# wangjunchi/LLMSeg

Hardware: AMD Instinct MI355X
Metric: images/sec (1024x1024, 64-tok prompt) model_forward fwd+bwd (higher is better)
Workload: dtype bf16; 1 GPU; BASELINE.json configs[2]: synthetic 1024x1024 + random-init LLaVA-7B(Llama-7B+CLIP-L/14)/SAM-ViT-H, batch_size=2 per GPU, fwd+bwd train step (CE + align + IoP losses, LoRA r=8 dropout 0.05 on q/v + trainable embed/lm_head/text_fcs/lisa_*, frozen towers, fp32 gradient arena, AdamW step every 10 micro-steps inside the timed region, micro-step replayed from a hipGraph), 256 candidate masks, 64-token ; global_batch=2, parallelism=dp1, graph=True, valid=True

## Files before the change

include/llmseg_hip.h:

```cpp
#ifndef LLMSEG_HIP_H
#define LLMSEG_HIP_H

#include <stdint.h>

#ifdef __cplusplus
extern "C" {
#endif

#define LLMSEG_OK 0
#define LLMSEG_EINVAL (-1)
#define LLMSEG_ELAUNCH (-2)
#define LLMSEG_NOT_TAKEN 1

enum { LLMSEG_ACT_NONE = 0, LLMSEG_ACT_RELU = 1, LLMSEG_ACT_GELU = 2, LLMSEG_ACT_QUICKGELU = 3, LLMSEG_ACT_SILU = 4,
       LLMSEG_ACT_SIGMOID = 5 };

#define LLMSEG_ABI_VERSION 14

#define LLMSEG_REDUCE_WS_BYTES (16 << 20)
int llmseg_version(void);
int64_t llmseg_launch_count(void);
int64_t llmseg_struct_size(int which);
const char* llmseg_last_error(void);

typedef struct {
  uint32_t struct_size;
  uint32_t reserved0;
  const void* A; const void* W; void* C;
  const void* bias;
  const void* gamma;
  const void* residual;
  int64_t M, N, K;
  int64_t lda, ldw, ldc, ldr;
  int64_t batch, strideA, strideW, strideC;
  float alpha;
  int act;
  int out_f32;
  int trans_a;
  int trans_w;
  int64_t batch2, strideA2, strideW2, strideC2;
  const void* A2; const void* W2; int64_t lda2, ldw2;
  void* workspace; int64_t workspace_bytes;
  int accumulate;
  const void* a_norm_w; float a_norm_eps; int a_swiglu;
  const void* norm_w; float norm_eps; int reserved1; void* norm_out; int64_t ldn;
  int fx; int fx_T; int64_t fx_cols; const float* fx_cos; const float* fx_sin; void* fx_out; const void* fx_in; int64_t fx_ld;
  const void* nb_x; const void* nb_w; const void* nb_dres; float nb_eps; int nb_rms;
  const void* nb_lora_t; int64_t nb_lora_ldt; const void* nb_lora_w0; const void* nb_lora_w1; float nb_lora_alpha; int reserved2; const void* nb_lora_drop;
  const void* dl_o; int64_t dl_ldo; float* dl_out; int32_t dl_heads; int32_t dl_T;
  const float* nb_lora_part; int32_t nb_lora_S; float nb_lora_scale; int32_t nb_lora_zero; int32_t reserved3;
// ... 161 lines not shown
                      int32_t* n_chars, int32_t cap_chars, void* workspace, int64_t workspace_bytes, void* stream);
int64_t llmseg_rle_parse_ws_bytes(int32_t K, int64_t total_chars);
int llmseg_rle_parse(const uint8_t* chars, const int64_t* char_offsets, int32_t K, uint32_t* run_ends, int64_t* run_offsets, void* workspace,
                     int64_t workspace_bytes, void* stream);

int llmseg_colsum(const void* x, float* out, int64_t M, int64_t N, int64_t ld, void* workspace, int64_t workspace_bytes, void* stream);
int llmseg_norm_bwd(const void* dy, const void* x, const void* w, void* dx, float* dw, float* db, int64_t rows, int64_t cols,
                    float eps, int rms, void* workspace, int64_t workspace_bytes, void* stream);
int llmseg_norm_bwd_add(const void* dy, const void* x, const void* w, const void* dres, void* dx, float* dw, float* db, int64_t rows, int64_t cols,
                        float eps, int rms, void* workspace, int64_t workspace_bytes, void* stream);
int llmseg_swiglu_bwd(const void* gu, const void* dout, void* dgu, int64_t rows, int64_t I, void* stream);
int llmseg_act_bwd(const void* dy, const void* y, void* out, int64_t n, int act, void* stream);
int llmseg_linear_bwd(const void* dy, const void* y, int act, const void* x, const void* w, void* dx, float* dw, float* db, int64_t M, int64_t N, int64_t K,
                      int accumulate, void* stream);
int llmseg_softmax_rows(const float* S, void* P, int64_t BH, int32_t Tq, int32_t Tk, int32_t ld, float scale, int32_t causal,
                        const uint8_t* key_mask, int32_t heads, void* stream);
int llmseg_attn_ds(const void* P, const float* dP, void* dS, int64_t rows, int32_t T, int32_t ld, float scale, void* stream);
int llmseg_ce_bwd(const void* logits, const int64_t* labels, const float* coef, void* dlogits, int32_t N, int32_t T, int64_t V,
                  int64_t ldl, void* stream);
int llmseg_scatter_add_rows(const void* src, const int64_t* idx, float* dst, int64_t n, int64_t cols, void* stream);
typedef struct {
  const uint64_t* rng_state;
  uint32_t stream;
  uint32_t drop_thr;
  uint32_t seg_rows;
  uint32_t reserved0;
} llmseg_dropout;
int llmseg_lora_down(const void* x0, const void* x1, int64_t ldx, const void* w0, const void* w1, void* y, int64_t ldy, int64_t M, int64_t K,
                     int32_t w_kr, float alpha, int32_t zero_cols, const llmseg_dropout* drop, void* stream);
int llmseg_lora_down_ws(const void* x0, const void* x1, int64_t ldx, const void* w0, const void* w1, void* y, int64_t ldy, int64_t M, int64_t K,
                        int32_t w_kr, float alpha, int32_t zero_cols, const llmseg_dropout* drop, void* scratch, int64_t scratch_bytes, void* stream);
int llmseg_lora_outer(const void* a0, const void* a1, int64_t lda, const void* b0, const void* b1, int64_t ldb, float* out0, float* out1, int64_t M,
                      int64_t N, int32_t out_rn, float alpha, const llmseg_dropout* drop, void* workspace, int64_t workspace_bytes, void* stream);
int llmseg_lora_wgrads(const void* dq, const void* dv, int64_t ldd, const void* x, int64_t ldx, const void* xa, int64_t ldxa, const void* t, int64_t ldt,
                       float* gbq, float* gbv, float* gaq, float* gav, int64_t M, int64_t H, float s, const llmseg_dropout* drop, void* workspace,
                       int64_t workspace_bytes, void* stream);
int llmseg_lora_apply(void* y, int64_t ldy, const void* xa, int64_t ldxa, const void* w0, const void* w1, int64_t M, int64_t N, int32_t w_rn,
                      float alpha, const llmseg_dropout* drop, void* stream);
int llmseg_lora_pack(const void* aq, const void* bq, const void* av, const void* bv, void* w2b, void* w2a, void* bt, int64_t H, float s, void* stream);
int llmseg_lora_down_parts(const void* x0, const void* x1, int64_t ldx, const void* w0, const void* w1, void* y, int64_t ldy, int64_t M, int64_t K,
                           int32_t w_kr, float alpha, int32_t zero_cols, const llmseg_dropout* drop, void* scratch, int64_t scratch_bytes, int32_t* S_out,
                           float* scale_out, void* stream);
int llmseg_lora_down_pack(const void* x0, const void* x1, int64_t ldx, const void* w0, const void* w1, void* y, int64_t ldy, int64_t M, int64_t K,
                          int32_t w_kr, float alpha, int32_t zero_cols, const llmseg_dropout* drop, void* scratch, int64_t scratch_bytes, const void* aq,
                          const void* bq, const void* av, const void* bv, void* w2b, void* w2a, void* bt, int64_t H, float s, void* stream);
int llmseg_transpose_pad(const void* in, void* out, int64_t rows, int64_t cols, int64_t ld_in, int64_t ld_out, int64_t rows_pad, void* stream);
int llmseg_sumsq(const void* x, int64_t n, int is_f32, float* out, void* workspace, int64_t workspace_bytes, void* stream);
int llmseg_adamw(void* p, float* master, const void* grad, int grad_f32, float* m, float* v, int64_t n, float lr, float beta1,
                 float beta2, float eps, float weight_decay, int64_t step, const float* grad_scale, void* stream);

int llmseg_prof_enable(int on);
const char* llmseg_prof_dominant_kernel(void);
double llmseg_prof_dominant_bytes(void);
int llmseg_prof_dominant_info(int64_t* out4);
int llmseg_prof_collect(double* total_ms, double* total_flops, int64_t* launches, double* dom_ms, double* dom_flops, int64_t* dom_launches);

#ifdef __cplusplus
}
#endif
#endif
```

llmseg_amd/_lib.py:

```python
import ctypes as C
import os

_HERE = os.path.dirname(os.path.abspath(__file__))
LIB_PATH = os.environ.get("LLMSEG_LIB") or os.path.join(_HERE, "libllmseg_hip.so")

ABI_VERSION = 14

ACT_NONE, ACT_RELU, ACT_GELU, ACT_QUICKGELU, ACT_SILU, ACT_SIGMOID = range(6)
NOT_TAKEN = 1


class _Sized(C.Structure):

    def __init__(self, *a, **kw):
        super().__init__(*a, **kw)
        self.struct_size = C.sizeof(self)


class GemmArgs(_Sized):
    _fields_ = [("struct_size", C.c_uint32), ("reserved0", C.c_uint32), ("A", C.c_void_p), ("W", C.c_void_p), ("C", C.c_void_p),
                ("bias", C.c_void_p), ("gamma", C.c_void_p), ("residual", C.c_void_p),
                ("M", C.c_int64), ("N", C.c_int64), ("K", C.c_int64),
                ("lda", C.c_int64), ("ldw", C.c_int64), ("ldc", C.c_int64), ("ldr", C.c_int64),
                ("batch", C.c_int64), ("strideA", C.c_int64), ("strideW", C.c_int64), ("strideC", C.c_int64),
                ("alpha", C.c_float), ("act", C.c_int), ("out_f32", C.c_int), ("trans_a", C.c_int), ("trans_w", C.c_int),
                ("batch2", C.c_int64), ("strideA2", C.c_int64), ("strideW2", C.c_int64), ("strideC2", C.c_int64),
                ("A2", C.c_void_p), ("W2", C.c_void_p), ("lda2", C.c_int64), ("ldw2", C.c_int64),
                ("workspace", C.c_void_p), ("workspace_bytes", C.c_int64), ("accumulate", C.c_int),
                ("a_norm_w", C.c_void_p), ("a_norm_eps", C.c_float), ("a_swiglu", C.c_int),
                ("norm_w", C.c_void_p), ("norm_eps", C.c_float), ("reserved1", C.c_int), ("norm_out", C.c_void_p), ("ldn", C.c_int64),
                ("fx", C.c_int), ("fx_T", C.c_int), ("fx_cols", C.c_int64), ("fx_cos", C.c_void_p), ("fx_sin", C.c_void_p), ("fx_out", C.c_void_p),
                ("fx_in", C.c_void_p), ("fx_ld", C.c_int64),
                ("nb_x", C.c_void_p), ("nb_w", C.c_void_p), ("nb_dres", C.c_void_p), ("nb_eps", C.c_float), ("nb_rms", C.c_int),
                ("nb_lora_t", C.c_void_p), ("nb_lora_ldt", C.c_int64), ("nb_lora_w0", C.c_void_p), ("nb_lora_w1", C.c_void_p), ("nb_lora_alpha", C.c_float),
                ("reserved2", C.c_int), ("nb_lora_drop", C.c_void_p),
                ("dl_o", C.c_void_p), ("dl_ldo", C.c_int64), ("dl_out", C.c_void_p), ("dl_heads", C.c_int32), ("dl_T", C.c_int32),
                ("nb_lora_part", C.c_void_p), ("nb_lora_S", C.c_int32), ("nb_lora_scale", C.c_float), ("nb_lora_zero", C.c_int32), ("reserved3", C.c_int32)]

class GemmW8Args(_Sized):
# ... 78 lines not shown
    "llmseg_cosine_scores": [_p, _p, _p, _i32, _i32, _p],
    "llmseg_linear_f32": [_p, _i64, _p, _i64, _i32, _p, _p, _i64, _p, _i64, _i32, _i32, _i32, _i32, _f32, _p],
    "llmseg_layernorm_f32": [_p, _p, _p, _p, _i64, _i32, _f32, _p],
    "llmseg_attn_f32": [_p, _p, _p, _p, C.POINTER(C.c_int64), _i32, _i32, _i32, _i32, _i32, _f32, _p],
    "llmseg_cosine_f32": [_p, _p, _p, _i32, _i32, _p],
    "llmseg_align_reg_loss": [_p, _p, _p, _p, _p, _p, _p, _p, _p, _i32, _i32, _f32, _i32, _p],
    "llmseg_dice_bce": [_p, _p, _p, _i32, _i64, _f32, _p, _i64, _p],
    "llmseg_dice_bce_bwd": [_p, _p, _p, _p, _i32, _i64, _f32, _p],
    "llmseg_ce_loss": [_p, _p, _p, _i32, _i32, _i64, _i64, _p, _i64, _p],
    "llmseg_intersection_union": [_p, _p, _i64, _i32, _p, _p],
    "llmseg_union_resize_iou": [_p, _p, _p, _i32, _i32, _i32, _i32, _i32, _i32, _i32, _i32, _p, _p],
    "llmseg_rle_decode": [_p, _p, _p, _i32, _i32, _i32, _i32, _p],
    "llmseg_rle_encode_ws_bytes": [_i32, _i32, _i32],
    "llmseg_rle_encode": [_p, _i32, _i32, _i32, _p, _p, _i32, _p, _p, _i32, _p, _i64, _p],
    "llmseg_rle_parse_ws_bytes": [_i32, _i64],
    "llmseg_rle_parse": [_p, _p, _i32, _p, _p, _p, _i64, _p],
    "llmseg_mask_targets": [_p, _p, _p, _p, _i32, _i32, _i32, _i32, _i32, _p, _p, _p, _p, _p],
    "llmseg_gt_resample": [_p, _p, _p, _p, _i32, _i32, _i32, _i32, _p],
    "llmseg_proposal_targets": [_p, _p, _p, _i32, _p, _i32, _i32, _i32, _i32, _p, _p, _p, _p, _p, _p, _i32, _p, _p, _p, _p, _p],
    "llmseg_resize_aa": [_p, _p, _i32, _i32, _i32, _i32, _p, _p, _p, _p, _p, _p, _i32, _p],
    "llmseg_colsum": [_p, _p, _i64, _i64, _i64, _p, _i64, _p],
    "llmseg_norm_bwd": [_p, _p, _p, _p, _p, _p, _i64, _i64, _f32, C.c_int, _p, _i64, _p],
    "llmseg_norm_bwd_add": [_p, _p, _p, _p, _p, _p, _p, _i64, _i64, _f32, C.c_int, _p, _i64, _p],
    "llmseg_swiglu_bwd": [_p, _p, _p, _i64, _i64, _p],
    "llmseg_act_bwd": [_p, _p, _p, _i64, C.c_int, _p],
    "llmseg_linear_bwd": [_p, _p, C.c_int, _p, _p, _p, _p, _p, _i64, _i64, _i64, C.c_int, _p],
    "llmseg_softmax_rows": [_p, _p, _i64, _i32, _i32, _i32, _f32, _i32, _p, _i32, _p],
    "llmseg_attn_ds": [_p, _p, _p, _i64, _i32, _i32, _f32, _p],
    "llmseg_ce_bwd": [_p, _p, _p, _p, _i32, _i32, _i64, _i64, _p],
    "llmseg_scatter_add_rows": [_p, _p, _p, _i64, _i64, _p],
    "llmseg_lora_down": [_p, _p, _i64, _p, _p, _p, _i64, _i64, _i64, _i32, _f32, _i32, _dp, _p],
    "llmseg_lora_down_ws": [_p, _p, _i64, _p, _p, _p, _i64, _i64, _i64, _i32, _f32, _i32, _dp, _p, _i64, _p],
    "llmseg_lora_outer": [_p, _p, _i64, _p, _p, _i64, _p, _p, _i64, _i64, _i32, _f32, _dp, _p, _i64, _p],
    "llmseg_lora_wgrads": [_p, _p, _i64, _p, _i64, _p, _i64, _p, _i64, _p, _p, _p, _p, _i64, _i64, _f32, _dp, _p, _i64, _p],
    "llmseg_lora_apply": [_p, _i64, _p, _i64, _p, _p, _i64, _i64, _i32, _f32, _dp, _p],
    "llmseg_lora_pack": [_p, _p, _p, _p, _p, _p, _p, _i64, _f32, _p],
    "llmseg_lora_down_parts": [_p, _p, _i64, _p, _p, _p, _i64, _i64, _i64, _i32, _f32, _i32, _dp, _p, _i64, C.POINTER(C.c_int32), C.POINTER(C.c_float), _p],
    "llmseg_lora_down_pack": [_p, _p, _i64, _p, _p, _p, _i64, _i64, _i64, _i32, _f32, _i32, _dp, _p, _i64, _p, _p, _p, _p, _p, _p, _p, _i64, _f32, _p],
    "llmseg_transpose_pad": [_p, _p, _i64, _i64, _i64, _i64, _i64, _p],
    "llmseg_sumsq": [_p, _i64, C.c_int, _p, _p, _i64, _p],
    "llmseg_adamw": [_p, _p, _p, C.c_int, _p, _p, _i64, _f32, _f32, _f32, _f32, _f32, _i64, _p, _p],
    "llmseg_prof_enable": [C.c_int],
    "llmseg_prof_dominant_kernel": [],
    "llmseg_prof_dominant_bytes": [],
    "llmseg_prof_dominant_info": [C.POINTER(C.c_int64)],
    "llmseg_prof_collect": [C.POINTER(C.c_double), C.POINTER(C.c_double), C.POINTER(C.c_int64), C.POINTER(C.c_double), C.POINTER(C.c_double),
                            C.POINTER(C.c_int64)],
}

_lib = None


def load():
    global _lib
    if _lib is not None:
        return _lib
    if not os.path.exists(LIB_PATH):
        raise RuntimeError(f"{LIB_PATH} not found: the HIP extension is not built "
                           f"(run llmseg_amd/csrc/build.sh); there is no CPU fallback")
    lib = C.CDLL(LIB_PATH)
    for name, argtypes in SIGNATURES.items():
        fn = getattr(lib, name)
        fn.argtypes = argtypes
        fn.restype = (C.c_char_p if name in ("llmseg_last_error", "llmseg_prof_dominant_kernel") else
                      C.c_double if name == "llmseg_prof_dominant_bytes" else C.c_int64 if name in ("llmseg_struct_size", "llmseg_launch_count", "llmseg_image_resize_workspace", "llmseg_mask_small_regions_workspace",
                                                                                            "llmseg_image_resize_filter_workspace", "llmseg_clip_preprocess_workspace",
# ... 14 lines not shown
```

llmseg_amd/csrc/backward.hip:

```cpp
#include <algorithm>
#include <cstdlib>
#include "common.h"
#include "llmseg_hip.h"

namespace {

inline unsigned grid_for(long total) {
  long g = (total + 255) / 256;
  return (unsigned)(g < 1 ? 1 : (g > 8192 ? 8192 : g));
}

__global__ __launch_bounds__(256) void colsum_kernel(const bf16_t* __restrict__ x, float* __restrict__ out, float* __restrict__ part, long M, long N, long ld) {
  __shared__ float red[4][64];
  const int c = threadIdx.x & 63, rl = threadIdx.x >> 6;
  const long col = (long)blockIdx.x * 64 + c;
  const long rows_per = (M + gridDim.y - 1) / gridDim.y;
  const long r0 = (long)blockIdx.y * rows_per, r1 = min(M, r0 + rows_per);
  float s = 0.f;
  if (col < N)
    for (long r = r0 + rl; r < r1; r += 4) s += bf2f(x[r * ld + col]);
  red[rl][c] = s;
  __syncthreads();
  if (rl == 0 && col < N) {
    const float v = (red[0][c] + red[1][c]) + (red[2][c] + red[3][c]);
// ... 688 lines not shown
    *reinterpret_cast<uint4*>(y + (m0 + mm) * ldy + ch * 8) = o;
  }
}

__device__ __forceinline__ void lora_down_finish_body(const float* __restrict__ part, int S, bf16_t* __restrict__ y, long ldy, long M, float scale,
                                                      int zero_cols, int nb, long bid, long nblocks) {
  const int nch = nb + zero_cols / 8;
  const long total = M * nch;
  for (long t = bid * blockDim.x + threadIdx.x; t < total; t += nblocks * blockDim.x) {
    const long mm = t / nch;
    const int ch = (int)(t - mm * nch);
    uint4 o = make_uint4(0, 0, 0, 0);
    if (ch < nb) {
      float v[8];
#pragma unroll
      for (int e = 0; e < 8; ++e) v[e] = 0.f;
      for (int s2 = 0; s2 < S; ++s2) {
        const float* pp = part + ((long)s2 * M + mm) * 16 + ch * 8;
#pragma unroll
        for (int e = 0; e < 8; ++e) v[e] += pp[e];
      }
#pragma unroll
      for (int e = 0; e < 8; ++e) v[e] *= scale;
      o = pack8(v);
    }
    *reinterpret_cast<uint4*>(y + mm * ldy + ch * 8) = o;
  }
}
__global__ __launch_bounds__(256) void lora_down_finish_kernel(const float* __restrict__ part, int S, bf16_t* __restrict__ y, long ldy, long M, float scale,
                                                              int zero_cols, int nb) {
  lora_down_finish_body(part, S, y, ldy, M, scale, zero_cols, nb, blockIdx.x, gridDim.x);
}

struct OuterP { const bf16_t* a[4]; const bf16_t* b[4]; float* out[4]; long lda[4], ldb[4]; int out_rn[4]; float alpha[4]; uint32_t drop[4]; };
__global__ __launch_bounds__(256) void lora_outer_kernel(OuterP q, long M, long N, DropP dp, float* __restrict__ part) {
  __shared__ float red[4][8][8 * LR];
  const int z = blockIdx.z;
  const bf16_t* __restrict__ a = q.a[z];
  const bf16_t* __restrict__ b = q.b[z];
  float* __restrict__ out = q.out[z];
  const long lda = q.lda[z], ldb = q.ldb[z];
  const int out_rn = q.out_rn[z];
  const float alpha = q.alpha[z];
  if (q.drop[z] == 0) dp.thr = 0;
  const uint32_t dstream = q.drop[z] - 1;
  const int lane = threadIdx.x & 63, wave = threadIdx.x >> 6;
  const int cl = lane & 7, rl = lane >> 3;
  const long n = ((long)blockIdx.x * 8 + cl) * 8;
  const long per = (M + gridDim.y * 4 - 1) / (gridDim.y * 4);
  const long m0 = ((long)blockIdx.y * 4 + wave) * per, m1 = min(M, m0 + per);
  const bool on = n < N;
  float acc[8][LR];
#pragma unroll
  for (int j = 0; j < 8; ++j)
#pragma unroll
    for (int r = 0; r < LR; ++r) acc[j][r] = 0.f;
  if (on) {
    long m = m0 + rl;
    for (; m + 16 < m1; m += 24) {
      uint4 av[3], bv[3];
#pragma unroll
      for (int u = 0; u < 3; ++u) {
        av[u] = *reinterpret_cast<const uint4*>(a + (m + 8 * u) * lda + n);
        bv[u] = *reinterpret_cast<const uint4*>(b + (m + 8 * u) * ldb);
      }
#pragma unroll
      for (int u = 0; u < 3; ++u) {
        float x[8], y[8];
        unpack8(av[u], x); unpack8(bv[u], y);
        if (dp.thr) {
          uint32_t oa;
          const unsigned long di = drop_index(dp, (unsigned long)(m + 8 * u), (unsigned long)N, (unsigned long)n, oa);
          dropout8(x, di, dstream, dp.rng, dp.thr, dp.scale, oa);
        }
#pragma unroll
        for (int j = 0; j < 8; ++j)
#pragma unroll
          for (int r = 0; r < LR; ++r) acc[j][r] = fmaf(x[j], y[r], acc[j][r]);
      }
    }
    for (; m < m1; m += 8) {
      float x[8], y[8];
      unpack8(*reinterpret_cast<const uint4*>(a + m * lda + n), x);
      unpack8(*reinterpret_cast<const uint4*>(b + m * ldb), y);
      if (dp.thr) {
        uint32_t oa;
        const unsigned long di = drop_index(dp, (unsigned long)m, (unsigned long)N, (unsigned long)n, oa);
        dropout8(x, di, dstream, dp.rng, dp.thr, dp.scale, oa);
      }
#pragma unroll
      for (int j = 0; j < 8; ++j)
#pragma unroll
        for (int r = 0; r < LR; ++r) acc[j][r] = fmaf(x[j], y[r], acc[j][r]);
    }
  }
#pragma unroll
  for (int j = 0; j < 8; ++j)
#pragma unroll
    for (int r = 0; r < LR; ++r) {
      float v = acc[j][r];
      v += __shfl_xor(v, 8, 64); v += __shfl_xor(v, 16, 64); v += __shfl_xor(v, 32, 64);
      acc[j][r] = v * alpha;
    }
  if (rl == 0) {
#pragma unroll
    for (int j = 0; j < 8; ++j)
#pragma unroll
      for (int r = 0; r < LR; ++r) red[wave][cl][j * LR + r] = acc[j][r];
  }
  __syncthreads();
  float* __restrict__ dstp = part ? part + ((long)blockIdx.y * gridDim.z + z) * N * LR : out;
  for (int idx = threadIdx.x; idx < 8 * 8 * LR; idx += blockDim.x) {
    const int c = idx / (8 * LR), jr = idx % (8 * LR), j = jr / LR, r = jr % LR;
    const long nn = ((long)blockIdx.x * 8 + c) * 8 + j;
    if (nn < N) {
      const float v = (red[0][c][jr] + red[1][c][jr]) + (red[2][c][jr] + red[3][c][jr]);
      const long cell = out_rn ? (long)r * N + nn : nn * LR + r;
      if (part) dstp[cell] = v;
      else dstp[cell] += v;
    }
  }
}

__global__ __launch_bounds__(256) void lora_apply_kernel(bf16_t* __restrict__ y, long ldy, const bf16_t* __restrict__ xa, long ldxa,
                                                        const bf16_t* __restrict__ w0, const bf16_t* __restrict__ w1, long M, long N, int w_rn,
                                                        float alpha, int nb, DropP dp) {
  const long nch = N >> 3, total = M * nch;
  for (long i = (long)blockIdx.x * blockDim.x + threadIdx.x; i < total; i += (long)gridDim.x * blockDim.x) {
    const long m = i / nch, c = i % nch;
    float yv[8], wv[8];
    unpack8(*reinterpret_cast<const uint4*>(y + m * ldy + c * 8), yv);
    for (int b = 0; b < nb; ++b) {
      const bf16_t* w = b == 0 ? w0 : w1;
      float xv[8], dv[8];
      unpack8(*reinterpret_cast<const uint4*>(xa + m * ldxa + 8 * b), xv);
      if (w_rn) {
#pragma unroll
        for (int j = 0; j < 8; ++j) dv[j] = 0.f;
#pragma unroll
        for (int r = 0; r < LR; ++r) {
          unpack8(*reinterpret_cast<const uint4*>(w + (long)r * N + c * 8), wv);
#pragma unroll
          for (int j = 0; j < 8; ++j) dv[j] += xv[r] * wv[j];
        }
      } else {
#pragma unroll
        for (int j = 0; j < 8; ++j) {
          unpack8(*reinterpret_cast<const uint4*>(w + (c * 8 + j) * LR), wv);
          float s = 0.f;
#pragma unroll
          for (int r = 0; r < LR; ++r) s += xv[r] * wv[r];
          dv[j] = s;
        }
      }
// ... 210 lines not shown
           "lora_down: bad arguments");
  const DropP dp = make_drop(drop);
  const bf16_t *X0 = (const bf16_t*)x0, *X1 = (const bf16_t*)(x1 ? x1 : x0), *W0 = (const bf16_t*)w0, *W1 = (const bf16_t*)(w1 ? w1 : w0);
  static const int force = getenv("LLMSEG_LORA_DOWN") ? atoi(getenv("LLMSEG_LORA_DOWN")) : 0;
  if (!w_kr && (K & 127) == 0 && force != 1) {
    if (force == 2) scratch = nullptr;
    const long tiles = (M + 15) / 16;
    int S = 1;
    while (tiles * S < 256 && (K % (4 * 32 * S * 2)) == 0 && scratch && (int64_t)S * 2 * M * 16 * 4 <= scratch_bytes && S < 32) S *= 2;
    float* part = S > 1 ? (float*)scratch : nullptr;
    LL_LAUNCH_KERNEL(lora_down_mfma_kernel, dim3((unsigned)tiles, (unsigned)S), dim3(256), 0, (hipStream_t)stream, X0, X1, (long)ldx, W0, W1, (bf16_t*)y, (long)ldy,
                       (long)M, (int)K, alpha, zero_cols, nb, dp, part);
    if (S > 1 && g_parts_req.active) {
      g_parts_req.done = true; g_parts_req.S = S; g_parts_req.scale = alpha * (dp.thr ? dp.scale : 1.f);
    } else if (S > 1 && g_pack_req.active) {
      const PackReq& q = g_pack_req;
      const unsigned gf = grid_for(M * (nb + zero_cols / 8)), gp = grid_for(4 * q.H * 8 + 2 * q.H);
      LL_LAUNCH_KERNEL(lora_finish_pack_kernel, dim3(gf + gp), dim3(256), 0, (hipStream_t)stream, (const float*)part, S, (bf16_t*)y, (long)ldy, (long)M,
                         alpha * (dp.thr ? dp.scale : 1.f), zero_cols, nb, (int)gf, q.aq, q.bq, q.av, q.bv, q.w2b, q.w2a, q.bt, q.H, q.s);
      g_pack_req.done = true;
    } else if (S > 1)
      LL_LAUNCH_KERNEL(lora_down_finish_kernel, dim3(grid_for(M * (nb + zero_cols / 8))), dim3(256), 0, (hipStream_t)stream, (const float*)part, S, (bf16_t*)y,
                         (long)ldy, (long)M, alpha * (dp.thr ? dp.scale : 1.f), zero_cols, nb);
  } else if (M <= 2048)
    LL_LAUNCH_KERNEL(lora_down_kernel<1>, dim3((unsigned)((M + 3) / 4)), dim3(256), 0, (hipStream_t)stream, X0, X1, (long)ldx, W0, W1, (bf16_t*)y, (long)ldy, (long)M,
                       (int)K, w_kr, alpha, zero_cols, nb, dp);
  else
    LL_LAUNCH_KERNEL(lora_down_kernel<4>, dim3((unsigned)((M + 15) / 16)), dim3(256), 0, (hipStream_t)stream, X0, X1, (long)ldx, W0, W1, (bf16_t*)y, (long)ldy, (long)M,
                       (int)K, w_kr, alpha, zero_cols, nb, dp);
  LL_LAUNCH_CHECK("lora_down");
  return LLMSEG_OK;
}

static int lora_outer_launch(const OuterP& q, int nz, int64_t M, int64_t N, const DropP& dp, void* workspace, int64_t workspace_bytes, hipStream_t stream) {
  const long colwg = (N + 63) / 64;
  long gy = max(max((long)1, 256 / (colwg * nz)), min((long)32, M / 512));
  gy = min(gy, workspace ? (long)(workspace_bytes / (nz * N * LR * 4)) : 0L);
  float* part = gy > 1 ? (float*)workspace : nullptr;
  if (gy < 1) gy = 1;
  LL_LAUNCH_KERNEL(lora_outer_kernel, dim3((unsigned)colwg, (unsigned)gy, (unsigned)nz), dim3(256), 0, stream, q, (long)M, (long)N, dp, part);
  if (part)
    LL_LAUNCH_KERNEL(fold_slices_kernel, dim3(fold_grid(nz * N * LR)), dim3(256), 0, stream, (const float*)part, (int)gy, (long)(nz * N * LR),
                     (long)(nz * N * LR), (long)(N * LR), FoldOut{{q.out[0], q.out[1], q.out[2], q.out[3]}});
  LL_LAUNCH_CHECK("lora_outer");
  return LLMSEG_OK;
}

extern "C" int llmseg_lora_outer(const void* a0, const void* a1, int64_t lda, const void* b0, const void* b1, int64_t ldb, float* out0, float* out1, int64_t M,
                                 int64_t N, int32_t out_rn, float alpha, const llmseg_dropout* drop, void* workspace, int64_t workspace_bytes, void* stream) {
  const int nz = (a1 && b1 && out1) ? 2 : 1;
  LL_CHECK(a0 && b0 && out0 && ((!a1) == (!b1)) && ((!a1) == (!out1)) && M > 0 && N > 0 && (N & 7) == 0 && (lda & 7) == 0 && (ldb & 7) == 0 && AL16(a0) &&
               AL16(a1) && AL16(b0) && AL16(b1) && LL_DROP_OK(drop), "lora_outer: bad arguments (N, lda, ldb multiples of 8)");
  OuterP q{};
  const DropP dp = make_drop(drop);
  for (int z = 0; z < nz; ++z) {
    q.a[z] = (const bf16_t*)(z ? a1 : a0); q.b[z] = (const bf16_t*)(z ? b1 : b0); q.out[z] = z ? out1 : out0;
    q.lda[z] = lda; q.ldb[z] = ldb; q.out_rn[z] = out_rn; q.alpha[z] = alpha; q.drop[z] = dp.thr ? dp.stream + z + 1 : 0;
  }
  return lora_outer_launch(q, nz, M, N, dp, workspace, workspace_bytes, (hipStream_t)stream);
}

extern "C" int llmseg_lora_wgrads(const void* dq, const void* dv, int64_t ldd, const void* x, int64_t ldx, const void* xa, int64_t ldxa, const void* t,
                                  int64_t ldt, float* gbq, float* gbv, float* gaq, float* gav, int64_t M, int64_t H, float s, const llmseg_dropout* drop,
                                  void* workspace, int64_t workspace_bytes, void* stream) {
  LL_CHECK(dq && dv && x && xa && t && gbq && gbv && gaq && gav && M > 0 && H > 0 && (H & 7) == 0 && (ldd & 7) == 0 && (ldx & 7) == 0 && (ldxa & 7) == 0 &&
               (ldt & 7) == 0 && ldxa >= 16 && ldt >= 16 && AL16(dq) && AL16(dv) && AL16(x) && AL16(xa) && AL16(t) && LL_DROP_OK(drop),
           "lora_wgrads: bad arguments");
  const DropP dp = make_drop(drop);
  OuterP q{};
  q.a[0] = (const bf16_t*)dq; q.b[0] = (const bf16_t*)xa;     q.out[0] = gbq; q.lda[0] = ldd; q.ldb[0] = ldxa; q.out_rn[0] = 0; q.alpha[0] = s;   q.drop[0] = 0;
  q.a[1] = (const bf16_t*)dv; q.b[1] = (const bf16_t*)xa + 8; q.out[1] = gbv; q.lda[1] = ldd; q.ldb[1] = ldxa; q.out_rn[1] = 0; q.alpha[1] = s;   q.drop[1] = 0;
  q.a[2] = (const bf16_t*)x;  q.b[2] = (const bf16_t*)t;      q.out[2] = gaq; q.lda[2] = ldx; q.ldb[2] = ldt;  q.out_rn[2] = 1; q.alpha[2] = 1.f; q.drop[2] = dp.thr ? dp.stream + 1 : 0;
  q.a[3] = (const bf16_t*)x;  q.b[3] = (const bf16_t*)t + 8;  q.out[3] = gav; q.lda[3] = ldx; q.ldb[3] = ldt;  q.out_rn[3] = 1; q.alpha[3] = 1.f; q.drop[3] = dp.thr ? dp.stream + 2 : 0;
// ... 252 lines not shown
```

llmseg_amd/csrc/common.h:

```cpp
#pragma once
#include "llmseg_hip.h"
#include <hip/hip_runtime.h>
#include <stdint.h>

typedef uint16_t bf16_t;
typedef __bf16 bf16x8_t __attribute__((ext_vector_type(8)));
typedef float f32x16_t __attribute__((ext_vector_type(16)));
typedef float f32x4_t __attribute__((ext_vector_type(4)));

__device__ __forceinline__ float bf2f(bf16_t v) { return __uint_as_float(((uint32_t)v) << 16); }

__device__ __forceinline__ bf16_t f2bf(float f) {
  uint32_t u = __float_as_uint(f);
  if ((u & 0x7fffffffu) > 0x7f800000u) return (bf16_t)((u >> 16) | 0x40);
  u += 0x7fffu + ((u >> 16) & 1u);
  return (bf16_t)(u >> 16);
}
typedef __bf16 bf16x2_t __attribute__((ext_vector_type(2)));
typedef float f32x2_t __attribute__((ext_vector_type(2)));
__device__ __forceinline__ uint32_t pack2bf(float lo, float hi) {
  const f32x2_t v = {lo, hi};
  return __builtin_bit_cast(uint32_t, __builtin_convertvector(v, bf16x2_t));
}

// ... 68 lines not shown
}

struct CeRow {
  uint2 q[32];
  __device__ __forceinline__ void load(const bf16_t* __restrict__ row, long V) {
    const long nq = V >> 2;
#pragma unroll
    for (int i = 0; i < 32; ++i) {
      const long k = threadIdx.x + 256L * i;
      q[i] = k < nq ? *reinterpret_cast<const uint2*>(row + 4 * k) : make_uint2(0xff80ff80u, 0xff80ff80u);
    }
  }
  __device__ __forceinline__ void stats(float* red, float& mx, float& s) const {
    float m = -1e30f;
#pragma unroll
    for (int i = 0; i < 32; ++i) {
      m = fmaxf(m, fmaxf(__uint_as_float(q[i].x << 16), __uint_as_float(q[i].x & 0xffff0000u)));
      m = fmaxf(m, fmaxf(__uint_as_float(q[i].y << 16), __uint_as_float(q[i].y & 0xffff0000u)));
    }
    mx = block_max(m, red);
    float t = 0.f;
#pragma unroll
    for (int i = 0; i < 32; ++i)
      t += __expf(__uint_as_float(q[i].x << 16) - mx) + __expf(__uint_as_float(q[i].x & 0xffff0000u) - mx) +
           __expf(__uint_as_float(q[i].y << 16) - mx) + __expf(__uint_as_float(q[i].y & 0xffff0000u) - mx);
    s = block_sum(t, red);
  }
};
__device__ __forceinline__ bool ce_row_fast(const bf16_t* row, long V, long ldl) {
  return V <= 32768 && (V & 3) == 0 && (ldl & 3) == 0 && (((uintptr_t)row) & 7) == 0 && blockDim.x == 256;
}

struct Philox8 { uint32_t w[4]; };
__device__ __forceinline__ Philox8 philox4x32_10(uint32_t c0, uint32_t c1, uint32_t c2, uint32_t c3, uint32_t k0, uint32_t k1) {
#pragma unroll
  for (int r = 0; r < 10; ++r) {
    const uint32_t hi0 = __umulhi(0xD2511F53u, c0), lo0 = 0xD2511F53u * c0;
    const uint32_t hi1 = __umulhi(0xCD9E8D57u, c2), lo1 = 0xCD9E8D57u * c2;
    c0 = hi1 ^ c1 ^ k0; c1 = lo1; c2 = hi0 ^ c3 ^ k1; c3 = lo0;
    k0 += 0x9E3779B9u; k1 += 0xBB67AE85u;
  }
  return Philox8{{c0, c1, c2, c3}};
}
__device__ __forceinline__ void dropout8(float* f, unsigned long idx, uint32_t stream, const unsigned long* rng, uint32_t thr, float scale, uint32_t off_add = 0) {
  const unsigned long seed = rng[0], off = rng[1] + off_add;
  const Philox8 r = philox4x32_10((uint32_t)idx, (uint32_t)(idx >> 32), stream, (uint32_t)off, (uint32_t)seed, (uint32_t)(seed >> 32));
#pragma unroll
  for (int j = 0; j < 8; ++j) {
    const uint32_t field = (r.w[j >> 1] >> (16 * (j & 1))) & 0xffffu;
    f[j] = field >= thr ? f[j] * scale : 0.f;
  }
}


struct FoldOut { float* p[4]; };
static __global__ __launch_bounds__(256) void fold_slices_kernel(const float* __restrict__ part, int P, long pstride, long n, long n0, FoldOut outs) {
  for (long i = (long)blockIdx.x * blockDim.x + threadIdx.x; i < n; i += (long)gridDim.x * blockDim.x) {
    const long seg = i / n0;
    float* o = outs.p[seg];
    if (!o) continue;
    float s = 0.f;
    for (int p = 0; p < P; ++p) s += part[(long)p * pstride + i];
    o[i - seg * n0] += s;
  }
}
static __global__ __launch_bounds__(256) void fold_column_kernel(const float* __restrict__ part, long P, float* __restrict__ out, float scale) {
  __shared__ float red[16];
  const long n = gridDim.x, i = blockIdx.x;
  float s = 0.f;
  for (long p = threadIdx.x; p < P; p += 256) s += part[p * n + i];
  s = block_sum(s, red);
  if (threadIdx.x == 0) out[i] += scale * s;
}
static inline unsigned fold_grid(long n) { const long g = (n + 255) / 256; return (unsigned)(g < 1 ? 1 : (g > 2048 ? 2048 : g)); }

void llmseg_count_launch();
#define LL_LAUNCH_KERNEL(...)              \
  do {                                     \
    llmseg_count_launch();                 \
    hipLaunchKernelGGL(__VA_ARGS__);       \
  } while (0)

void llmseg_set_error(const char* fmt, ...);
void llmseg_prof_begin(hipStream_t s);
// ... 26 lines not shown
```

Before: 51.86 images/s.

## Add streaming LoRA outer-product kernel with register prefetch pipeline

Adds a new default kernel for the LoRA outer-product weight gradient. It keeps D rows of A and B in registers as a software-pipelined prefetch, steps the dropout segment index incrementally instead of dividing per row, and uses 64-bit multiplies for Philox. It also loads the existing output values before the main loop so the final accumulate needs no read-modify-write. The old kernel stays available through an environment variable or a set_variant call, and is used automatically for negative strides. The aim is to hide global-load latency in a bandwidth-bound reduction over M, at the cost of higher register pressure under launch_bounds(256,2).

Result: no change. 51.96 images/s, median of 6 (+0.2%).

```diff
diff --git a/include/llmseg_hip.h b/include/llmseg_hip.h
--- a/include/llmseg_hip.h
+++ b/include/llmseg_hip.h
@@ -15,7 +15,7 @@
 enum { LLMSEG_ACT_NONE = 0, LLMSEG_ACT_RELU = 1, LLMSEG_ACT_GELU = 2, LLMSEG_ACT_QUICKGELU = 3, LLMSEG_ACT_SILU = 4,
        LLMSEG_ACT_SIGMOID = 5 };
 
-#define LLMSEG_ABI_VERSION 14
+#define LLMSEG_ABI_VERSION 15
 
 #define LLMSEG_REDUCE_WS_BYTES (16 << 20)
 int llmseg_version(void);
@@ -243,6 +243,7 @@
                         int32_t w_kr, float alpha, int32_t zero_cols, const llmseg_dropout* drop, void* scratch, int64_t scratch_bytes, void* stream);
 int llmseg_lora_outer(const void* a0, const void* a1, int64_t lda, const void* b0, const void* b1, int64_t ldb, float* out0, float* out1, int64_t M,
                       int64_t N, int32_t out_rn, float alpha, const llmseg_dropout* drop, void* workspace, int64_t workspace_bytes, void* stream);
+int llmseg_lora_outer_set_variant(int variant);
 int llmseg_lora_wgrads(const void* dq, const void* dv, int64_t ldd, const void* x, int64_t ldx, const void* xa, int64_t ldxa, const void* t, int64_t ldt,
                        float* gbq, float* gbv, float* gaq, float* gav, int64_t M, int64_t H, float s, const llmseg_dropout* drop, void* workspace,
                        int64_t workspace_bytes, void* stream);
diff --git a/llmseg_amd/_lib.py b/llmseg_amd/_lib.py
--- a/llmseg_amd/_lib.py
+++ b/llmseg_amd/_lib.py
@@ -4,7 +4,7 @@
 _HERE = os.path.dirname(os.path.abspath(__file__))
 LIB_PATH = os.environ.get("LLMSEG_LIB") or os.path.join(_HERE, "libllmseg_hip.so")
 
-ABI_VERSION = 14
+ABI_VERSION = 15
 
 ACT_NONE, ACT_RELU, ACT_GELU, ACT_QUICKGELU, ACT_SILU, ACT_SIGMOID = range(6)
 NOT_TAKEN = 1
@@ -149,6 +149,7 @@
     "llmseg_lora_down": [_p, _p, _i64, _p, _p, _p, _i64, _i64, _i64, _i32, _f32, _i32, _dp, _p],
     "llmseg_lora_down_ws": [_p, _p, _i64, _p, _p, _p, _i64, _i64, _i64, _i32, _f32, _i32, _dp, _p, _i64, _p],
     "llmseg_lora_outer": [_p, _p, _i64, _p, _p, _i64, _p, _p, _i64, _i64, _i32, _f32, _dp, _p, _i64, _p],
+    "llmseg_lora_outer_set_variant": [C.c_int],
     "llmseg_lora_wgrads": [_p, _p, _i64, _p, _i64, _p, _i64, _p, _i64, _p, _p, _p, _p, _i64, _i64, _f32, _dp, _p, _i64, _p],
     "llmseg_lora_apply": [_p, _i64, _p, _i64, _p, _p, _i64, _i64, _i32, _f32, _dp, _p],
     "llmseg_lora_pack": [_p, _p, _p, _p, _p, _p, _p, _i64, _f32, _p],
diff --git a/llmseg_amd/csrc/backward.hip b/llmseg_amd/csrc/backward.hip
--- a/llmseg_amd/csrc/backward.hip
+++ b/llmseg_amd/csrc/backward.hip
@@ -744,6 +744,51 @@
   lora_down_finish_body(part, S, y, ldy, M, scale, zero_cols, nb, blockIdx.x, gridDim.x);
 }
 
+__device__ __forceinline__ long lora_outer_cell(int idx, int out_rn, long N) {
+  const int c = idx / (8 * LR), jr = idx % (8 * LR), j = jr / LR, r = jr % LR;
+  const long nn = ((long)blockIdx.x * 8 + c) * 8 + j;
+  return nn < N ? (out_rn ? (long)r * N + nn : nn * LR + r) : -1;
+}
+__device__ __forceinline__ void lora_outer_prefetch(float (&prev)[2], const float* __restrict__ out, int out_rn, long N) {
+#pragma unroll
+  for (int k = 0; k < 2; ++k) {
+    const long cell = lora_outer_cell(threadIdx.x + 256 * k, out_rn, N);
+    prev[k] = out[cell >= 0 ? cell : 0];
+  }
+}
+template <bool PRE = false>
+__device__ __forceinline__ void lora_outer_fold_store(float (&acc)[8][LR], float (&red)[4][8][8 * LR], float alpha, float* __restrict__ out, int out_rn, long N,
+                                                      float* __restrict__ part, int z, const float* prev = nullptr) {
+  const int lane = threadIdx.x & 63, wave = threadIdx.x >> 6;
+  const int cl = lane & 7, rl = lane >> 3;
+#pragma unroll
+  for (int j = 0; j < 8; ++j)
+#pragma unroll
+    for (int r = 0; r < LR; ++r) {
+      float v = acc[j][r];
+      v += __shfl_xor(v, 8, 64); v += __shfl_xor(v, 16, 64); v += __shfl_xor(v, 32, 64);
+      acc[j][r] = v * alpha;
+    }
+  if (rl == 0) {
+#pragma unroll
+    for (int j = 0; j < 8; ++j)
+#pragma unroll
+      for (int r = 0; r < LR; ++r) red[wave][cl][j * LR + r] = acc[j][r];
+  }
+  __syncthreads();
+  float* __restrict__ dstp = part ? part + ((long)blockIdx.y * gridDim.z + z) * N * LR : out;
+  for (int idx = threadIdx.x, k = 0; idx < 8 * 8 * LR; idx += blockDim.x, ++k) {
+    const int c = idx / (8 * LR), jr = idx % (8 * LR);
+    const long cell = lora_outer_cell(idx, out_rn, N);
+    if (cell >= 0) {
+      const float v = (red[0][c][jr] + red[1][c][jr]) + (red[2][c][jr] + red[3][c][jr]);
+      if (part) dstp[cell] = v;
+      else if (PRE) dstp[cell] = prev[k] + v;
+      else dstp[cell] += v;
+    }
+  }
+}
+
 struct OuterP { const bf16_t* a[4]; const bf16_t* b[4]; float* out[4]; long lda[4], ldb[4]; int out_rn[4]; float alpha[4]; uint32_t drop[4]; };
 __global__ __launch_bounds__(256) void lora_outer_kernel(OuterP q, long M, long N, DropP dp, float* __restrict__ part) {
   __shared__ float red[4][8][8 * LR];
@@ -806,32 +851,97 @@
         for (int r = 0; r < LR; ++r) acc[j][r] = fmaf(x[j], y[r], acc[j][r]);
     }
   }
+  lora_outer_fold_store(acc, red, alpha, out, out_rn, N, part, z);
+}
+
+#ifndef LLMSEG_LORA_OUTER_D
+#define LLMSEG_LORA_OUTER_D 6
+#endif
+#ifndef LLMSEG_LORA_OUTER_WIDE
+#define LLMSEG_LORA_OUTER_WIDE 1
+#endif
+template <int D, bool DROP>
+__device__ __forceinline__ void lora_outer_stream_rows(float (&acc)[8][LR], const bf16_t* __restrict__ a, const bf16_t* __restrict__ b, long lda, long ldb, long m0,
+                                                       long m1, int rl, long n, long N, const DropP& dp, uint32_t dstream) {
+  const long mr = m0 + rl, mlast = m1 - 1;
+  const long steps = (m1 - m0 + 7) >> 3;
+  const bf16_t* const pa_last = a + mlast * lda + n;
+  const bf16_t* const pb_last = b + mlast * ldb;
+  const bf16_t* pa = a + min(mr, mlast) * lda + n;
+  const bf16_t* pb = b + min(mr, mlast) * ldb;
+  const long sa = 8 * lda, sb = 8 * ldb;
+  unsigned long seed = 0, off = 0, ml = (unsigned long)mr, seg = ~0ul, r8 = 8;
+  uint32_t sg = 0, q8 = 0;
+  if (DROP) {
+    seed = dp.rng[0]; off = dp.rng[1];
+    if (dp.seg) {
+      seg = dp.seg; q8 = 8 / dp.seg; r8 = 8 % dp.seg;
+      sg = (uint32_t)(ml / seg); ml -= (unsigned long)sg * seg;
+    }
+  }
+  uint4 av[D], bv[D];
+  auto fetch = [&](uint4& au, uint4& bu) {
+    au = *reinterpret_cast<const uint4*>(pa);
+    bu = *reinterpret_cast<const uint4*>(pb);
+    pa = pa + sa < pa_last ? pa + sa : pa_last;
+    pb = pb + sb < pb_last ? pb + sb : pb_last;
+  };
+  auto step = [&](const uint4& au, const uint4& bu) {
+    float x[8], y[8];
+    unpack8(au, x); unpack8(bu, y);
+    if (DROP) {
+      dropout8_at<LLMSEG_LORA_OUTER_WIDE != 0>(x, (ml * (unsigned long)N + (unsigned long)n) >> 3, dstream, seed, off + sg, dp.thr, dp.scale);
+      ml += r8; sg += q8;
+      if (ml >= seg) { ml -= seg; ++sg; }
+    }
+#pragma unroll
+    for (int j = 0; j < 8; ++j)
+#pragma unroll
+      for (int r = 0; r < LR; ++r) acc[j][r] = fmaf(x[j], y[r], acc[j][r]);
+#pragma unroll
+    for (int j = 0; j < 8; ++j)
+      asm volatile("" : "+v"(acc[j][0]), "+v"(acc[j][1]), "+v"(acc[j][2]), "+v"(acc[j][3]), "+v"(acc[j][4]), "+v"(acc[j][5]), "+v"(acc[j][6]), "+v"(acc[j][7]));
+  };
+#pragma unroll
+  for (int s = 0; s < D; ++s) fetch(av[s], bv[s]);
+  long base = 0;
+  for (; base + D < steps; base += D) {
+#pragma unroll
+    for (int s = 0; s < D; ++s) {
+      step(av[s], bv[s]);
+      fetch(av[s], bv[s]);
+      __builtin_amdgcn_sched_barrier(0);
+    }
+  }
+#pragma unroll
+  for (int s = 0; s < D; ++s)
+    if (mr + 8 * (base + s) < m1) step(av[s], bv[s]);
+}
+template <int D>
+__global__ __launch_bounds__(256, 2) void lora_outer_stream_kernel(OuterP q, long M, long N, DropP dp, float* __restrict__ part) {
+  __shared__ float red[4][8][8 * LR];
+  const int z = blockIdx.z;
+  const bf16_t* __restrict__ a = q.a[z];
+  const bf16_t* __restrict__ b = q.b[z];
+  const long lda = q.lda[z], ldb = q.ldb[z];
+  const uint32_t dstream = q.drop[z] - 1;
+  const int lane = threadIdx.x & 63, wave = __builtin_amdgcn_readfirstlane(threadIdx.x >> 6);
+  const int cl = lane & 7, rl = lane >> 3;
+  const long n = ((long)blockIdx.x * 8 + cl) * 8;
+  const long per = (M + gridDim.y * 4 - 1) / (gridDim.y * 4);
+  const long m0 = ((long)blockIdx.y * 4 + wave) * per, m1 = min(M, m0 + per);
+  float prev[2] = {0.f, 0.f};
+  if (!part) lora_outer_prefetch(prev, q.out[z], q.out_rn[z], N);
+  float acc[8][LR];
 #pragma unroll
   for (int j = 0; j < 8; ++j)
 #pragma unroll
-    for (int r = 0; r < LR; ++r) {
-      float v = acc[j][r];
-      v += __shfl_xor(v, 8, 64); v += __shfl_xor(v, 16, 64); v += __shfl_xor(v, 32, 64);
-      acc[j][r] = v * alpha;
-    }
-  if (rl == 0) {
-#pragma unroll
-    for (int j = 0; j < 8; ++j)
-#pragma unroll
-      for (int r = 0; r < LR; ++r) red[wave][cl][j * LR + r] = acc[j][r];
-  }
-  __syncthreads();
-  float* __restrict__ dstp = part ? part + ((long)blockIdx.y * gridDim.z + z) * N * LR : out;
-  for (int idx = threadIdx.x; idx < 8 * 8 * LR; idx += blockDim.x) {
-    const int c = idx / (8 * LR), jr = idx % (8 * LR), j = jr / LR, r = jr % LR;
-    const long nn = ((long)blockIdx.x * 8 + c) * 8 + j;
-    if (nn < N) {
-      const float v = (red[0][c][jr] + red[1][c][jr]) + (red[2][c][jr] + red[3][c][jr]);
-      const long cell = out_rn ? (long)r * N + nn : nn * LR + r;
-      if (part) dstp[cell] = v;
-      else dstp[cell] += v;
-    }
-  }
+    for (int r = 0; r < LR; ++r) acc[j][r] = 0.f;
+  if (n < N && m0 < m1) {
+    if (q.drop[z] != 0 && dp.thr) lora_outer_stream_rows<D, true>(acc, a, b, lda, ldb, m0, m1, rl, n, N, dp, dstream);
+    else lora_outer_stream_rows<D, false>(acc, a, b, lda, ldb, m0, m1, rl, n, N, dp, dstream);
+  }
+  lora_outer_fold_store<true>(acc, red, q.alpha[z], q.out[z], q.out_rn[z], N, part, z, prev);
 }
 
 __global__ __launch_bounds__(256) void lora_apply_kernel(bf16_t* __restrict__ y, long ldy, const bf16_t* __restrict__ xa, long ldxa,
@@ -1108,13 +1218,26 @@
   return LLMSEG_OK;
 }
 
+static int& lora_outer_variant() {
+  static int v = [] { const char* e = getenv("LLMSEG_LORA_OUTER_V1"); return (e && atoi(e) != 0) ? 1 : 0; }();
+  return v;
+}
+extern "C" int llmseg_lora_outer_set_variant(int variant) {
+  LL_CHECK(variant == 0 || variant == 1, "lora_outer_set_variant: 0 (streaming form) or 1 (the three-step form)");
+  lora_outer_variant() = variant;
+  return LLMSEG_OK;
+}
+
 static int lora_outer_launch(const OuterP& q, int nz, int64_t M, int64_t N, const DropP& dp, void* workspace, int64_t workspace_bytes, hipStream_t stream) {
   const long colwg = (N + 63) / 64;
   long gy = max(max((long)1, 256 / (colwg * nz)), min((long)32, M / 512));
   gy = min(gy, workspace ? (long)(workspace_bytes / (nz * N * LR * 4)) : 0L);
   float* part = gy > 1 ? (float*)workspace : nullptr;
   if (gy < 1) gy = 1;
-  LL_LAUNCH_KERNEL(lora_outer_kernel, dim3((unsigned)colwg, (unsigned)gy, (unsigned)nz), dim3(256), 0, stream, q, (long)M, (long)N, dp, part);
+  bool v1 = lora_outer_variant() == 1;
+  for (int z = 0; z < nz; ++z) v1 = v1 || q.lda[z] < 0 || q.ldb[z] < 0;
+  if (v1) LL_LAUNCH_KERNEL(lora_outer_kernel, dim3((unsigned)colwg, (unsigned)gy, (unsigned)nz), dim3(256), 0, stream, q, (long)M, (long)N, dp, part);
+  else LL_LAUNCH_KERNEL(lora_outer_stream_kernel<LLMSEG_LORA_OUTER_D>, dim3((unsigned)colwg, (unsigned)gy, (unsigned)nz), dim3(256), 0, stream, q, (long)M, (long)N, dp, part);
   if (part)
     LL_LAUNCH_KERNEL(fold_slices_kernel, dim3(fold_grid(nz * N * LR)), dim3(256), 0, stream, (const float*)part, (int)gy, (long)(nz * N * LR),
                      (long)(nz * N * LR), (long)(N * LR), FoldOut{{q.out[0], q.out[1], q.out[2], q.out[3]}});
diff --git a/llmseg_amd/csrc/common.h b/llmseg_amd/csrc/common.h
--- a/llmseg_amd/csrc/common.h
+++ b/llmseg_amd/csrc/common.h
@@ -124,24 +124,34 @@
 }
 
 struct Philox8 { uint32_t w[4]; };
+template <bool WIDE = false>
 __device__ __forceinline__ Philox8 philox4x32_10(uint32_t c0, uint32_t c1, uint32_t c2, uint32_t c3, uint32_t k0, uint32_t k1) {
 #pragma unroll
   for (int r = 0; r < 10; ++r) {
-    const uint32_t hi0 = __umulhi(0xD2511F53u, c0), lo0 = 0xD2511F53u * c0;
-    const uint32_t hi1 = __umulhi(0xCD9E8D57u, c2), lo1 = 0xCD9E8D57u * c2;
+    uint32_t hi0, lo0, hi1, lo1;
+    if (WIDE) {
+      const unsigned long p0 = (unsigned long)0xD2511F53u * c0, p1 = (unsigned long)0xCD9E8D57u * c2;
+      hi0 = (uint32_t)(p0 >> 32); lo0 = (uint32_t)p0; hi1 = (uint32_t)(p1 >> 32); lo1 = (uint32_t)p1;
+    } else {
+      hi0 = __umulhi(0xD2511F53u, c0); lo0 = 0xD2511F53u * c0;
+      hi1 = __umulhi(0xCD9E8D57u, c2); lo1 = 0xCD9E8D57u * c2;
+    }
     c0 = hi1 ^ c1 ^ k0; c1 = lo1; c2 = hi0 ^ c3 ^ k1; c3 = lo0;
     k0 += 0x9E3779B9u; k1 += 0xBB67AE85u;
   }
   return Philox8{{c0, c1, c2, c3}};
 }
-__device__ __forceinline__ void dropout8(float* f, unsigned long idx, uint32_t stream, const unsigned long* rng, uint32_t thr, float scale, uint32_t off_add = 0) {
-  const unsigned long seed = rng[0], off = rng[1] + off_add;
-  const Philox8 r = philox4x32_10((uint32_t)idx, (uint32_t)(idx >> 32), stream, (uint32_t)off, (uint32_t)seed, (uint32_t)(seed >> 32));
+template <bool WIDE = false>
+__device__ __forceinline__ void dropout8_at(float* f, unsigned long idx, uint32_t stream, unsigned long seed, unsigned long off, uint32_t thr, float scale) {
+  const Philox8 r = philox4x32_10<WIDE>((uint32_t)idx, (uint32_t)(idx >> 32), stream, (uint32_t)off, (uint32_t)seed, (uint32_t)(seed >> 32));
 #pragma unroll
   for (int j = 0; j < 8; ++j) {
     const uint32_t field = (r.w[j >> 1] >> (16 * (j & 1))) & 0xffffu;
     f[j] = field >= thr ? f[j] * scale : 0.f;
   }
+}
+__device__ __forceinline__ void dropout8(float* f, unsigned long idx, uint32_t stream, const unsigned long* rng, uint32_t thr, float scale, uint32_t off_add = 0) {
+  dropout8_at(f, idx, stream, rng[0], rng[1] + off_add, thr, scale);
 }
 
 
```
